# martinruenz/co-fusion

Hardware: AMD Instinct MI355X
Metric: frames/sec at 640x480 (N active models) + ICP-reduce achieved HBM GB/s vs peak (higher is better)
Workload: dtype f32

## Files before the change

### co_fusion_amd/csrc/cabi.hip

```cpp
#include <math.h>
#include <stdio.h>
#include <stdlib.h>
#include <string.h>

#include <string>
#include <vector>

#include "cf_host.h"
#include "gn_ref_host.h"

using namespace cf;

#define HIPCHK(ctx, call)                                                                      \
    do {                                                                                       \
        hipError_t e_ = (call);                                                                \
        if (e_ != hipSuccess) {                                                                \
            (ctx)->set_error(std::string(#call) + ": " + hipGetErrorString(e_));               \
            return CF_EHIP;                                                                    \
        }                                                                                      \
    } while (0)

#define LAUNCHCHK(ctx) HIPCHK(ctx, hipGetLastError())

void cf_ctx::set_error(const std::string& m)
// ... 641 lines not shown
    }
    LAUNCHCHK(ctx);
    return CF_OK;
}

static int populate_rgbd(cf_odom* od, const uint8_t* rgba, float* const* depths, uint8_t* const* images)
{
    cf_ctx* ctx = od->ctx; hipStream_t s = ctx->stream;
    RgbdBatch b{};
    b.c[0] = rgbd_chain(od, rgba, depths, images);
    launch_rgbd_pyramids(s, b, 1, ctx->cfg.width, ctx->cfg.height, od->maxDepthRGB);
    LAUNCHCHK(ctx);
    return CF_OK;
}
int cf_odom_init_rgb_model(cf_odom* od, const uint8_t* pred_rgba) { if (!od || !pred_rgba) return CF_EINVAL; return populate_rgbd(od, pred_rgba, od->lastDepth, od->lastImage); }
int cf_odom_init_rgb(cf_odom* od, const uint8_t* rgba) { if (!od || !rgba) return CF_EINVAL; od->next_depth_is_last = false; return populate_rgbd(od, rgba, od->nextDepth, od->nextImage); }

int cf_odom_init_models_batch(cf_ctx* ctx, cf_odom* const* ods, int n, const float* const* pred_v4, const float* const* pred_n4,
                              const uint8_t* const* pred_rgba, const float* const* poses, const uint8_t* frame_rgba)
{
    if (!ctx || n <= 0 || !frame_rgba) return CF_EINVAL;
    std::vector<const uint8_t*> frames((size_t)n, frame_rgba);
    return cf_odom_init_models_batch_frames(ctx, ods, n, pred_v4, pred_n4, pred_rgba, poses, frames.data());
}

int cf_odom_init_models_batch_frames(cf_ctx* ctx, cf_odom* const* ods, int n, const float* const* pred_v4, const float* const* pred_n4,
                                     const uint8_t* const* pred_rgba, const float* const* poses, const uint8_t* const* frame_rgba)
{
    return cf_odom_init_models_batch_select(ctx, ods, n, pred_v4, pred_n4, pred_rgba, nullptr, nullptr, nullptr, nullptr, 0.f, poses, frame_rgba);
}

// ... 23 lines not shown
        RgbdBatch rb{};
        for (int k = 0; k < nb; k++) {
            cf_odom* od = ods[base + k];
            if (!od || !pred_v4[base + k] || !pred_n4[base + k] || !pred_rgba[base + k] || !poses[base + k] || !frame_rgba[base + k]) return CF_EINVAL;
            mb.m[k] = model_maps_args(od, pred_v4[base + k], pred_n4[base + k], poses[base + k]);
            rb.c[k] = rgbd_chain(od, pred_rgba[base + k], od->lastDepth, od->lastImage);
            rb.c[k].v4 = pred_v4[base + k];
            if (choose && fill_counts[base + k]) {
                if (!alt_v4[base + k] || !alt_n4[base + k] || !alt_rgba[base + k]) return CF_EINVAL;
                mb.m[k].alt_v4 = alt_v4[base + k]; mb.m[k].alt_n4 = alt_n4[base + k]; mb.m[k].sel = fill_counts[base + k]; mb.m[k].sel_ratio = ratio;
                rb.c[k].alt_v4 = alt_v4[base + k]; rb.c[k].alt_rgba = alt_rgba[base + k]; rb.c[k].sel = fill_counts[base + k]; rb.c[k].sel_ratio = ratio;
            }
            od->next_depth_is_last = true;
        }
        int n_chains = nb;
        for (int k = 0; k < nb; k++) {
            cf_odom* od = ods[base + k];
            int owner = -1;
            for (int j = nb; j < n_chains; j++)
                if (rb.c[j].rgba == frame_rgba[base + k]) { owner = j; break; }
            if (owner < 0) {
                owner = n_chains++;
                rb.c[owner] = rgbd_chain(od, frame_rgba[base + k], od->nextDepth, od->nextImage);
                for (int i = 0; i < CF_NUM_PYRS; ++i) rb.c[owner].depth[i] = nullptr;
            }
            rb.fan_owner[k] = (signed char)(owner + 1);
            for (int i = 0; i < CF_NUM_PYRS; ++i) rb.fan_image[i][k] = od->nextImage[i];
        }
        launch_model_maps_and_pyramids(s, mb, nb, rb, n_chains, W, H, ods[base]->maxDepthRGB);
    }
    LAUNCHCHK(ctx);
    return CF_OK;
}

int cf_odom_init_first_rgb(cf_odom* od, const uint8_t* rgba)
{
    if (!od || !rgba) return CF_EINVAL;
    cf_ctx* ctx = od->ctx; hipStream_t s = ctx->stream;
    const int W = ctx->cfg.width, H = ctx->cfg.height;
    launch_intensity(s, rgba, W, H, od->lastNextImage[0]);
// ... 129 lines not shown
    const float t[3] = {pose[3], pose[7], pose[11]};
    memcpy(h->Rprev, R, 36); memcpy(h->tprev, t, 12); memcpy(h->Rcurr, R, 36); memcpy(h->tcurr, t, 12);
    inv33f_host(R, h->Rprev_inv);
    memset(&h->stats, 0, sizeof(h->stats));
    h->solves = 0;
    {
        const int its = (opts->fast_odom ? 3 : 10) + (opts->pyramid ? 9 : 0);
        od->expected_solves = its;
    }
    od->pending_so3_swap = opts->so3 != 0;
    od->launch_shape = LaunchShape{};
    LAUNCHCHK(ctx);
    return CF_OK;
}

static void fill_rgb_args(cf_ctx* ctx, cf_odom* const* ods, int n, RgbArgs out[3])
{
    const cf_cam intr{ctx->cfg.fx, ctx->cfg.fy, ctx->cfg.cx, ctx->cfg.cy};
    for (int l = 0; l < 3; l++) {
        RgbArgs& a = out[l];
        memset(&a, 0, sizeof(a));
        const int div = 1 << l;
        a.cols = ctx->cfg.width >> l; a.rows = ctx->cfg.height >> l;
        a.il = cf_cam{intr.fx / div, intr.fy / div, intr.cx / div, intr.cy / div};
        a.sobelScale = ods[0]->sobelScale; a.maxDepthDelta = ods[0]->maxDepthDeltaRGB;
        for (int m = 0; m < n; m++) {
            a.m[m] = rgb_model_args(ods[m]->h_state, ods[m]->d_state, l);
            a.m[m].no_counts = (ods[m]->band_end > 0 && !ods[m]->band_counts) ? 1 : 0;
            a.m[m].res_blocks = a.m[m].res_range ? residual_blocks_for(ods[m]->res_hint[l]) : 0;
        }
// ... 46 lines not shown
        }
    }
    if (ctx->icp_arith == CF_ICP_ARITH_REFERENCE) {
        for (int m = 0; m < n; m++)
            if (ods[m]->band_end > 0) { ctx->set_error("the reference-order arithmetic (cf_set_icp_arith 2) does not split a tracker's reductions over GPUs"); return CF_ESTATE; }
        RgbPrepBatch rp{};
        for (int base = 0; base < n; base += kPrepBatch) {
            const int nb = n - base < kPrepBatch ? n - base : kPrepBatch;
            rp = RgbPrepBatch{};
            for (int m = base; m < base + nb; m++) {
                if (int r = odom_prepare(ods[m], poses_in[m], opts, err_surfaces ? err_surfaces[m] : nullptr, &rp.m[m - base])) return r;
                ods[m]->h_state->cull = 0; ods[m]->h_state->res_range = nullptr; rp.m[m - base].res_range = nullptr;
                ods[m]->box_hint[0] = kNoBoxHint;
                HIPCHK(ctx, hipMemsetAsync(ods[m]->aabb, 0, 8 * sizeof(unsigned), ctx->stream));
            }
            if (want_rgb) launch_rgb_prep(ctx->stream, rp, nb, ctx->cfg.width, ctx->cfg.height);
        }
        LAUNCHCHK(ctx);
        for (int m = 0; m < n; m++)
            if (int r = ref_track(ctx, ods[m], poses_in[m], opts, err_surfaces ? err_surfaces[m] : nullptr)) return r;
        for (int m = 0; m < n; m++) ods[m]->result_pending = true;
        return CF_OK;
    }
    for (int m = 0; m < n; m++)
        if (ods[m]->gn_epoch_seen != ctx->gn_mode_epoch) {
            HIPCHK(ctx, hipMemsetAsync(ods[m]->rgb_acc, 0, sizeof(unsigned long long) * ods[m]->rgb_acc_words, ctx->stream));
            ods[m]->gn_epoch_seen = ctx->gn_mode_epoch;
        }
    const bool prep_fused = want_rgb && opts->so3 != 0 && n <= kPrepBatch;
    RgbPrepBatch prep{};
    for (int base = 0; base < n; base += kPrepBatch) {
        const int nb = n - base < kPrepBatch ? n - base : kPrepBatch;
        if (base) prep = RgbPrepBatch{};
        for (int m = base; m < base + nb; m++) {
            if (int r = odom_prepare(ods[m], poses_in[m], opts, err_surfaces ? err_surfaces[m] : nullptr, &prep.m[m - base])) return r;
        }
        if (want_rgb && !prep_fused) launch_rgb_prep(ctx->stream, prep, nb, ctx->cfg.width, ctx->cfg.height);
    }
    if (prep_fused) rgb_prep_levels(prep, n, ctx->cfg.width, ctx->cfg.height);
    TrackerStates states{};
    for (int m = 0; m < n; m++) { states.dev[m] = ods[m]->d_state; states.host[m] = ods[m]->h_state; }
    const bool so3_here = opts->so3 != 0;
    const bool icp = !opts->rgb_only && opts->icp_weight > 0;
    const bool rgb = opts->rgb_only || opts->icp_weight < 100;
    IcpArgs icp_args[3];
    fill_icp_args(ctx, ods, n, icp_args);
    RgbArgs rgb_args[3];
    fill_rgb_args(ctx, ods, n, rgb_args);
    OdomDev* h_states[kMaxBatch];
    for (int m = 0; m < n; m++) h_states[m] = ods[m]->h_state;
    GnHook hook{};
// ... 79 lines not shown
    if (!od) return CF_EINVAL;
    cf_ctx* ctx = od->ctx;
    if (int r = cf_wait_stream(ctx)) return r;
    od->result_pending = false;
    if (trans) memcpy(trans, od->h_state->tcurr, 12);
    if (rot) memcpy(rot, od->h_state->Rcurr, 36);
    if (stats) *stats = od->h_state->stats;
    bool fault = od->h_state->stats.fault != 0;
    if (ctx->icp_arith != CF_ICP_ARITH_REFERENCE && od->expected_solves >= 0 && od->h_state->solves != od->expected_solves) {
        (void)hipMemsetAsync(ctx->d_so3_sync, 0, sizeof(So3Sync) * ((size_t)ctx->cfg.max_models + 1), ctx->stream);
        fault = true;
    }
    od->expected_solves = -1;
    if (od->pending_so3_swap) {
        for (int i = 0; i < CF_NUM_PYRS; i++) std::swap(od->lastNextImage[i], od->nextImage[i]);
        od->pending_so3_swap = false;
    }
    if (fault) {
        ctx->set_error("tracking: a bounded device-side wait expired (workgroups of one launch were not co-resident)");
        return CF_ESTATE;
    }
    return CF_OK;
}

int cf_odom_get_covariance(const cf_track_stats* stats, double cov[36])
{
    if (!stats || !cov) return CF_EINVAL;
    constexpr int N = 6;
    double lu[N * N];
    int perm[N];
// ... 141 lines not shown
```

### co_fusion_amd/csrc/cf_host.h

```cpp
#pragma once

#include <mutex>
#include <string>

#include "cf_kernels.h"

struct cf_ctx;
struct cf_thread_binding { const cf_ctx* ctx = nullptr; hipStream_t stream = nullptr; };
extern thread_local cf_thread_binding cf_tls_binding;

struct cf_ctx {
    cf_config cfg{};
    hipStream_t stream = nullptr;
    hipStream_t cur() const { return cf_tls_binding.ctx == this ? cf_tls_binding.stream : stream; }
    hipStream_t own_stream = nullptr;
    std::string last_error;
    std::mutex error_mutex;
    cf::IcpLaunch icp_launch{256, 0};
    int icp_arith = 0;
    float* d_ref = nullptr;
    float* h_ref = nullptr;
    unsigned long long* d_acc_a = nullptr;
    unsigned long long* d_acc_b = nullptr;
    unsigned long long* d_out = nullptr;
    unsigned long long* h_out = nullptr;
    cf::OdomDev* d_scratch_state = nullptr;
    cf::OdomDev* h_scratch_state = nullptr;
    uint8_t* d_cand_scratch = nullptr;
    cf::So3Sync* d_so3_sync = nullptr;
    unsigned gn_mode_epoch = 0;
    int xcd_round_robin = -1;
    int gn_mode = 1;
    static constexpr int kStateSlots = 256;
    cf::OdomDev* d_state_pool = nullptr;
    cf::OdomDev* h_state_pool = nullptr;
    bool slot_used[kStateSlots]{};
    hipEvent_t batch_event = nullptr;
    static constexpr int kLanes = 8;
    hipStream_t lanes[kLanes]{};
    hipEvent_t lane_done[kLanes]{};
    hipEvent_t fork_point = nullptr;
    static constexpr int kMarks = 64;
    hipEvent_t marks[kMarks]{};
    bool mark_set[kMarks]{};
// ... 32 lines not shown
    float* nmap_g_prev[3]{};
    float* vmap_curr[3]{};
    float* nmap_curr[3]{};
    const float* ext_vmap_curr[3]{};
    const float* ext_nmap_curr[3]{};
    float2* zrange[3]{};
    bool zrange_valid = false;
    const float2* ext_zrange[3]{};
    float* lastDepth[3]{};
    float* nextDepth[3]{};
    bool next_depth_is_last = false;
    float* next_depth(int i) const { return next_depth_is_last ? lastDepth[i] : nextDepth[i]; }
    uint8_t* lastImage[3]{};
    uint8_t* nextImage[3]{};
    uint8_t* lastNextImage[3]{};
    int16_t* dIdx[3]{};
    int16_t* dIdy[3]{};
    float* cloud[3]{};
    cf_dataterm* corres[3]{};
    uint8_t* cand[3]{};
    unsigned char* occ = nullptr;
    bool occ_valid = false;
    bool use_occ = false;
    unsigned* aabb = nullptr;
    float map_pose[12]{};
    int box_hint[4] = {0x7fffffff, 0, 0, 0};
    unsigned* res_range = nullptr;
    int res_hint[3] = {-1, -1, -1};
    bool box_valid = false;
    int band_begin = 0, band_end = 0;
// ... 17 lines not shown
```

### co_fusion_amd/csrc/cf_kernels.h

```cpp
#pragma once

#include <hip/hip_runtime.h>
#include <hip/hip_ext.h>
#include <stdint.h>

#include "../../include/cofusion_hip.h"

namespace cf {

constexpr int kGroups = 64;

struct alignas(64) GnHot {
    int icp, level_done; float cull_z[2];
    float Rcurr[9], tcurr[3];
    float Rprev_inv[9], tprev[3];
    int cull_box[4];
    int rgb, rgbOnly, level_done2, pad;
    float krkInv[9], kt[3];
};
static_assert(sizeof(GnHot) == 192, "three 64-byte lines");

struct OdomDev;
struct OdomDev {
    const float* vmap_curr[3];
// ... 74 lines not shown
    const uint8_t* nextImage[3]; const float* nextDepth[3]; const float* lastDepth[3];
    int16_t* dIdx[3]; int16_t* dIdy[3]; uint8_t* cand[3]; float* cloud[3];
    float minScale[3], fx_inv[3], fy_inv[3], cx[3], cy[3];
    unsigned* res_range;
};
struct ModelMapsArgs {
    const float* pred_v4; const float* pred_n4;
    const float* alt_v4; const float* alt_n4;
    const unsigned* sel; float sel_ratio;
    float* snapshot;
    float* vmap[3]; float* nmap[3];
    int cols, rows;
    float R[9], t[3];
    unsigned char* occ;
    unsigned* aabb;
};
constexpr int kPrepBatch = 8;
struct ModelMapsBatch { ModelMapsArgs m[kPrepBatch]; };
struct RgbPrepBatch { RgbPrepArgs m[kPrepBatch]; };
struct RgbdChain {
    const float* v4; const uint8_t* rgba; float* depth[3]; uint8_t* image[3];
    const float* alt_v4; const uint8_t* alt_rgba; const unsigned* sel; float sel_ratio;
};
struct RgbdBatch {
    RgbdChain c[2 * kPrepBatch];
    uint8_t* fan_image[3][kPrepBatch];
    signed char fan_owner[kPrepBatch];
};
void launch_model_maps(hipStream_t s, const ModelMapsBatch& b, int n);
void launch_frame_maps(hipStream_t s, FrameMapsArgs a, int W, int H);
void launch_rgbd_pyramids(hipStream_t s, const RgbdBatch& b, int n_chains, int W, int H, float cutoff);
void launch_model_maps_and_pyramids(hipStream_t s, const ModelMapsBatch& mb, int n, const RgbdBatch& rb, int n_chains, int W, int H, float cutoff);
void launch_rgb_prep(hipStream_t s, RgbPrepBatch b, int n, int W, int H);

struct IDiv { unsigned M, s; };
inline IDiv make_idiv(int d)
{
    if (d < 2) return IDiv{0x80000000u, 0u};
    unsigned l = 0;
    while ((1u << l) < (unsigned)d) l++;
    return IDiv{(unsigned)((((unsigned long long)1 << (31 + l)) + (unsigned)d - 1) / (unsigned)d), l - 1};
}
constexpr int kGramBits[8] = {20, 20, 20, 17, 17, 17, 22, 0};
struct LaunchShape { int icp[3]; int res[3]; int icp_err; };
struct IcpLaunch { int threads; int ppt; int gram;
                   LaunchShape* const* shape = nullptr; };

// ... 218 lines not shown
```

### co_fusion_amd/csrc/track_prep.hip

```cpp
#include "cf_device.h"
#include "cf_kernels.h"
#include "track_prep_dev.h"

namespace cf {

static constexpr int kBlock = 256;
static inline int grid_for(int n) { return (n + kBlock - 1) / kBlock; }

__global__ void __launch_bounds__(kBlock) vmap_kernel(const float* __restrict__ depth, int cols, int rows, float fx_inv,
                                                      float fy_inv, float cx, float cy, float cutoff,
                                                      float* __restrict__ vmap)
{
    const int i = blockIdx.x * kBlock + threadIdx.x;
    if (i >= cols * rows) return;
    const int v = i / cols, u = i - v * cols;
    const float z = depth[i];
    if (z != 0 && z < cutoff) {
        vmap[i] = z * (u - cx) * fx_inv;
        vmap[i + rows * cols] = z * (v - cy) * fy_inv;
        vmap[i + 2 * rows * cols] = z;
    } else {
        vmap[i] = qnan();
    }
}
// ... 190 lines not shown
    const float4* __restrict__ v4 = reinterpret_cast<const float4*>(alt ? c.alt_v4 : c.v4);
    const uchar4* __restrict__ rgba = reinterpret_cast<const uchar4*>(alt ? c.alt_rgba : c.rgba);
    const int nb = (N + kBlock - 1) / kBlock;
    if (bx < nb) {
        const int i = bx * kBlock + threadIdx.x;
        if (i >= N || !c.depth[0]) return;
        const float z = v4[i].z;
        c.depth[0][i] = (z > cutoff || z <= 0) ? qnan() : z;
    } else {
        const int i = (bx - nb) * kBlock + threadIdx.x;
        if (i >= N) return;
        const uchar4 s = rgba[i];
        rgbd_store_image(b, by, 0, i, (uint8_t)(int)((float)s.x * 0.114f + (float)s.y * 0.299f + (float)s.z * 0.587f));
    }
}
__global__ void __launch_bounds__(kBlock) rgbd_base_kernel(const RgbdBatch b, int N, float cutoff) { rgbd_base_body(b, N, cutoff, (int)blockIdx.x, (int)blockIdx.y); }
__global__ void __launch_bounds__(kBlock) rgbd_pyrdown_kernel(const RgbdBatch b, int level, int scols, int srows)
{
    const RgbdChain& c = b.c[blockIdx.y];
    const int n = (scols / 2) * (srows / 2), nb = (n + kBlock - 1) / kBlock;
    if ((int)blockIdx.x < nb) {
        const int i = blockIdx.x * kBlock + threadIdx.x;
        if (i < n && c.depth[level]) pyrdown_f32_px(c.depth[level], scols, srows, c.depth[level + 1], i);
    } else {
        const int i = (blockIdx.x - nb) * kBlock + threadIdx.x;
        if (i < n) rgbd_store_image(b, (int)blockIdx.y, level + 1, i, pyrdown_u8_val(c.image[level], scols, srows, i));
    }
}

__global__ void __launch_bounds__(kBlock) rgb_expand_kernel(const uint8_t* __restrict__ rgb, int N, uchar4* __restrict__ rgba)
// ... 97 lines not shown
    }
    if (edge) { nmap[i] = qnan(); return; }
    const float x01 = (z01 != 0 && z01 < cutoff) ? z01 * ((u + 1) - cx) * fx_inv : qnan();
    const float x10 = (z10 != 0 && z10 < cutoff) ? z10 * (u - cx) * fx_inv : qnan();
    if (!is_nan(x00) && !is_nan(x01) && !is_nan(x10)) {
        const f3 v00 = {x00, z * (v - cy) * fy_inv, z};
        const f3 v01 = {x01, z01 * (v - cy) * fy_inv, z01};
        const f3 v10 = {x10, z10 * ((v + 1) - cy) * fy_inv, z10};
        const f3 r = normalized(cross(v01 - v00, v10 - v00));
        nmap[i] = r.x; nmap[i + N] = r.y; nmap[i + 2 * N] = r.z;
    } else {
        nmap[i] = qnan();
    }
}

__global__ void __launch_bounds__(kBlock) rgb_prep_kernel(const RgbPrepBatch b) { rgb_prep_body(b.m[blockIdx.y], (int)blockIdx.x); }

struct MapVal { f3 p; bool have; };

__device__ __forceinline__ void emit_map(float* __restrict__ map, int idx, int N, const MapVal& m, const m33& R, const f3& t, bool add_t)
{
    if (!m.have) { map[idx] = qnan(); return; }
    if (!is_nan(m.p.x)) {
        f3 d = mul(R, m.p);
        if (add_t) d = d + t;
        map[idx] = d.x; map[idx + N] = d.y; map[idx + 2 * N] = d.z;
    } else {
        map[idx] = qnan(); map[idx + N] = m.p.y; map[idx + 2 * N] = m.p.z;
    }
}

// ... 71 lines not shown
    const int cols = a.cols, rows = a.rows, N0 = cols * rows, c1 = cols >> 1, c2 = cols >> 2, N1 = N0 >> 2, N2 = N0 >> 4;
    const int lane = threadIdx.x & 63, lx = lane & 15, ly = lane >> 4;
    const int tiles_x = cols >> 4;
    const int tile = bx * 4 + (threadIdx.x >> 6);
    if (tile >= tiles_x * (rows >> 2)) return;
    const int ty = tile / tiles_x, tx = tile - ty * tiles_x;
    const int x = tx * 16 + lx, y = ty * 4 + ly, i0 = y * cols + x;
    const bool alt = a.sel && (float)a.sel[0] / (float)a.sel[1] < a.sel_ratio;
    const float4* __restrict__ v4 = reinterpret_cast<const float4*>(alt ? a.alt_v4 : a.pred_v4);
    const float4* __restrict__ n4 = reinterpret_cast<const float4*>(alt ? a.alt_n4 : a.pred_n4);
    float4* __restrict__ snap = reinterpret_cast<float4*>(a.snapshot);
    m33 R; for (int k = 0; k < 9; k++) R.m[k] = a.R[k];
    const f3 tr = {a.t[0], a.t[1], a.t[2]};
    const float4 vs = v4[i0], ns = n4[i0];
    snap[i0] = vs;
    MapVal v0, n0;
    v0.have = true; n0.have = true;
    const bool valid = !(vs.z == 0);
    if (valid) { v0.p = f3{vs.x, vs.y, vs.z}; n0.p = f3{ns.x, ns.y, ns.z}; }
    else { v0.p = f3{qnan(), qnan(), qnan()}; n0.p = v0.p; }
    emit_map(a.vmap[0], i0, N0, v0, R, tr, true);
    emit_map(a.nmap[0], i0, N0, n0, R, tr, false);
    const MapVal v01 = lane_mapval(v0, lane + 1), v10 = lane_mapval(v0, lane + 16), v11 = lane_mapval(v0, lane + 17);
    const MapVal n01 = lane_mapval(n0, lane + 1), n10 = lane_mapval(n0, lane + 16), n11 = lane_mapval(n0, lane + 17);
    MapVal v1, n1;
    v1.have = false; n1.have = false; v1.p = f3{qnan(), qnan(), qnan()}; n1.p = v1.p;
    if (((lx | ly) & 1) == 0) {
        v1 = resize4(v0, v01, v10, v11, false);
        n1 = resize4(n0, n01, n10, n11, true);
        const int i1 = (y >> 1) * c1 + (x >> 1);
// ... 15 lines not shown
        const float inf = __int_as_float(0x7f800000);
        float lo[3] = {inf, inf, inf}, hi[3] = {-inf, -inf, -inf};
        if (valid && !is_nan(v0.p.x) && !is_nan(vs.z)) { lo[0] = hi[0] = (float)x; lo[1] = hi[1] = (float)y; lo[2] = hi[2] = vs.z; }
#pragma unroll
        for (int o = 32; o > 0; o >>= 1)
#pragma unroll
            for (int k = 0; k < 3; k++) { lo[k] = fminf(lo[k], __shfl_xor(lo[k], o, 64)); hi[k] = fmaxf(hi[k], __shfl_xor(hi[k], o, 64)); }
        if (lane < 6 && lo[0] <= hi[0] && lo[1] <= hi[1] && lo[2] <= hi[2]) {
            const float val = lane == 0 ? lo[0] : lane == 1 ? lo[1] : lane == 2 ? lo[2] : lane == 3 ? hi[0] : lane == 4 ? hi[1] : hi[2];
            const unsigned key = lane < 3 ? ~fkey(val) : fkey(val);
            if (key > __hip_atomic_load(&a.aabb[lane], __ATOMIC_RELAXED, __HIP_MEMORY_SCOPE_AGENT)) atomicMax(&a.aabb[lane], key);
        }
    }
}
__global__ void __launch_bounds__(256) model_maps_tiled_kernel(const ModelMapsBatch b) { model_maps_tiled_body(b, (int)blockIdx.x, (int)blockIdx.y); }
__global__ void __launch_bounds__(256) prep_fused_kernel(const ModelMapsBatch mb, int mm_bx, int mm_total, const RgbdBatch rb, int N, float cutoff, int rb_bx)
{
    const int b = blockIdx.x;
    if (b < mm_total) { const int by = b / mm_bx; model_maps_tiled_body(mb, b - by * mm_bx, by); }
    else { const int r = b - mm_total, by = r / rb_bx; rgbd_base_body(rb, N, cutoff, r - by * rb_bx, by); }
}

static Level3 levels3(int W, int H)
{
    Level3 L; int acc = 0;
    for (int i = 0; i < 3; i++) { L.cols[i] = W >> i; L.rows[i] = H >> i; acc += grid_for(L.cols[i] * L.rows[i]); L.blk_end[i] = acc; }
    return L;
}
void launch_frame_maps(hipStream_t s, FrameMapsArgs a, int W, int H)
{
    a.L = levels3(W, H);
    frame_maps_kernel<<<a.L.blk_end[2], kBlock, 0, s>>>(a);
}
void rgb_prep_levels(RgbPrepBatch& b, int n, int W, int H)
{
    const Level3 L = levels3(W, H);
    for (int m = 0; m < n; m++) b.m[m].L = L;
}
void launch_rgb_prep(hipStream_t s, RgbPrepBatch b, int n, int W, int H)
{
    const Level3 L = levels3(W, H);
    for (int m = 0; m < n; m++) b.m[m].L = L;
    rgb_prep_kernel<<<dim3(L.blk_end[2], n), kBlock, 0, s>>>(b);
}
void launch_model_maps(hipStream_t s, const ModelMapsBatch& b, int n)
{
    const int cols = b.m[0].cols, rows = b.m[0].rows;
    if (cols % 16 == 0 && rows % 4 == 0) {
        const int tiles = (cols >> 4) * (rows >> 2);
        model_maps_tiled_kernel<<<dim3((tiles + 3) / 4, n), 256, 0, s>>>(b);
        return;
    }
    const int t = (cols >> 2) * (rows >> 2);
    model_maps_kernel<<<dim3((t + 63) / 64, n), 64, 0, s>>>(b);
}
void launch_model_maps_and_pyramids(hipStream_t s, const ModelMapsBatch& mb, int n, const RgbdBatch& rb, int n_chains, int W, int H, float cutoff)
{
    static_assert(kBlock == 256, "the fused launch runs both bodies with 256 threads");
    const int cols = mb.m[0].cols, rows = mb.m[0].rows;
    if (cols % 16 == 0 && rows % 4 == 0) {
        const int mm_bx = ((cols >> 4) * (rows >> 2) + 3) / 4, rb_bx = 2 * grid_for(W * H);
        prep_fused_kernel<<<mm_bx * n + rb_bx * n_chains, 256, 0, s>>>(mb, mm_bx, mm_bx * n, rb, W * H, cutoff, rb_bx);
    } else {
        launch_model_maps(s, mb, n);
        rgbd_base_kernel<<<dim3(2 * grid_for(W * H), n_chains), kBlock, 0, s>>>(rb, W * H, cutoff);
    }
    for (int i = 0; i + 1 < 3; i++)
        rgbd_pyrdown_kernel<<<dim3(2 * grid_for(((W >> i) / 2) * ((H >> i) / 2)), n_chains), kBlock, 0, s>>>(rb, i, W >> i, H >> i);
}
void launch_rgbd_pyramids(hipStream_t s, const RgbdBatch& b, int n_chains, int W, int H, float cutoff)
{
    rgbd_base_kernel<<<dim3(2 * grid_for(W * H), n_chains), kBlock, 0, s>>>(b, W * H, cutoff);
    for (int i = 0; i + 1 < 3; i++)
        rgbd_pyrdown_kernel<<<dim3(2 * grid_for(((W >> i) / 2) * ((H >> i) / 2)), n_chains), kBlock, 0, s>>>(b, i, W >> i, H >> i);
}
void launch_vmap(hipStream_t s, const float* depth, int cols, int rows, cf_cam intr, float cutoff, float* vmap)
{
// ... 55 lines not shown
```

### co_fusion_amd/csrc/track_prep_dev.h

```cpp
#pragma once
#include "cf_device.h"
#include "cf_kernels.h"

namespace cf {
__device__ __forceinline__ int level_of(const Level3& L, int b, int& lb)
{
    const int lv = b < L.blk_end[0] ? 0 : (b < L.blk_end[1] ? 1 : 2);
    lb = b - (lv ? L.blk_end[lv - 1] : 0);
    return lv;
}

__device__ __forceinline__ void rgb_prep_body(const RgbPrepArgs& a, int bx)
{
    int lb;
    const int lv = level_of(a.L, bx, lb);
    const int cols = a.L.cols[lv], rows = a.L.rows[lv];
    const int k = lb * 256 + (int)threadIdx.x;
    uint8_t ok = 0;
    if (k < cols * rows) {
    const int y = k / cols, x = k - y * cols;
    const uint8_t* __restrict__ src = a.nextImage[lv];
    {
        const float z = a.lastDepth[lv][k];
        float* __restrict__ cloud3 = a.cloud[lv];
        cloud3[k * 3 + 0] = (x - a.cx[lv]) * z * a.fx_inv[lv];
        cloud3[k * 3 + 1] = (y - a.cy[lv]) * z * a.fy_inv[lv];
        cloud3[k * 3 + 2] = z;
    }
    float dxv = 0, dyv = 0;
    constexpr float sx[9] = {0.52201f, 0.00000f, -0.52201f, 0.79451f, -0.00000f, -0.79451f, 0.52201f, 0.00000f, -0.52201f};
    constexpr float sy[9] = {0.52201f, 0.79451f, 0.52201f, 0.00000f, 0.00000f, 0.00000f, -0.52201f, -0.79451f, -0.52201f};
    if (x >= 1 && y >= 1 && x <= cols - 2 && y <= rows - 2) {
        const uint8_t* __restrict__ p0 = src + (y - 1) * cols + (x - 1);
#pragma unroll
        for (int r = 0; r < 3; r++)
#pragma unroll
            for (int c = 0; c < 3; c++) {
                const float s = (float)p0[r * cols + c];
                dxv += s * sx[8 - (r * 3 + c)];
                dyv += s * sy[8 - (r * 3 + c)];
            }
    } else {
        int kk = 8;
        for (int j = max(y - 1, 0); j <= min(y + 1, rows - 1); j++)
            for (int c = max(x - 1, 0); c <= min(x + 1, cols - 1); c++) {
                const float s = (float)src[j * cols + c];
                dxv += s * sx[kk];
                dyv += s * sy[kk];
                --kk;
            }
    }
    const int16_t dx16 = (int16_t)(int)dxv, dy16 = (int16_t)(int)dyv;
    a.dIdx[lv][k] = dx16; a.dIdy[lv][k] = dy16;
    if (x < cols - 5 && y < rows - 1) {
        bool valid = true;
        for (int u = max(y - 2, 0); u < min(y + 2, rows); u++)
            for (int v = max(x - 2, 0); v < min(x + 2, cols); v++) valid = valid && (src[u * cols + v] > 0);
        if (valid) {
            const int valx = dx16, valy = dy16;
            const float mTwo = (float)((valx * valx) + (valy * valy));
            if (mTwo >= a.minScale[lv] && !is_nan(a.nextDepth[lv][k])) ok = 1;
        }
    }
    a.cand[lv][k] = ok;
    }
    if (a.res_range) {
        if (__syncthreads_or(ok)) {
            if (threadIdx.x == 0) { atomicMax(&a.res_range[2 * lv], ~(unsigned)lb); atomicMax(&a.res_range[2 * lv + 1], (unsigned)lb + 1u); }
        }
    }
}
}
```

### co_fusion_amd/csrc/track_reduce.hip

```cpp
#include "cf_device.h"
#include "cf_kernels.h"
#include "track_prep_dev.h"
#include "track_sums_dev.h"

namespace cf {

__device__ __forceinline__ int idiv(int n, IDiv d) { return (int)(__umulhi((unsigned)n, d.M) >> d.s); }

struct IcpProj { f3 vcurr_g; int g; int inb; int ux, uy; };

__device__ __forceinline__ IcpProj icp_project(const m33& Rcurr, const f3& tcurr, const m33& Rprev_inv, const f3& tprev, const cf_cam& intr,
                                               int cols, int rows, f3 vcurr)
{
    IcpProj o;
    o.vcurr_g = mul(Rcurr, vcurr) + tcurr;
    const f3 vcurr_cp = mul(Rprev_inv, o.vcurr_g - tprev);
    const int ux = f2i_rn(vcurr_cp.x * intr.fx / vcurr_cp.z + intr.cx);
    const int uy = f2i_rn(vcurr_cp.y * intr.fy / vcurr_cp.z + intr.cy);
    o.inb = !(ux < 0 || uy < 0 || ux >= cols || uy >= rows || vcurr_cp.z < 0);
    o.g = o.inb ? uy * cols + ux : 0;
    o.ux = o.inb ? ux : 0; o.uy = o.inb ? uy : 0;
    return o;
}

// ... 672 lines not shown

bool launch_gn_track(hipStream_t s, IcpLaunch cfg, const TrackerStates& states, So3Sync* so3_syncs, const GnHook* hook, const IcpArgs icp_args[3],
                     const RgbArgs rgb_args[3], int n, int width, int height, bool so3, bool pyramid, bool fast_odom, bool rgb, bool icp, int mode,
                     ProfSink* prof, OdomDev* const* h_states, const RgbPrepBatch* prep)
{
    int iterations[3];
    iterations[0] = fast_odom ? 3 : 10;
    iterations[1] = pyramid ? 5 : 0;
    iterations[2] = pyramid ? 4 : 0;
    int first_level = 2;
    while (first_level > 0 && iterations[first_level] == 0) first_level--;
    {
        const int gx = so3 ? 8 * kSo3Blocks : 1;
        static const RgbPrepBatch none{};
        const int prep_bx = prep ? prep->m[0].L.blk_end[2] : 0;
        so3_prealign_kernel<<<gx * n + prep_bx * n, 256, 0, s>>>(states, so3_syncs, so3 ? 1 : 0, first_level, gx, gx * n, prep ? *prep : none, prep_bx);
    }
    GnArgs gn{};
    gn.icp_gram = cfg.gram;
    gn.slot_px = cfg.threads * 4;
    for (int m = 0; m < n; m++) {
        gn.od[m] = const_cast<OdomDev*>(icp_args[0].m[m].st);
        gn.icp_acc[m] = icp_args[0].m[m].acc;
        gn.rgb_acc[m] = rgb_args[0].m[m].rgb_acc;
        gn.od_host[m] = h_states ? h_states[m] : nullptr;
    }
    const bool slots = mode != 0;
    bool any_culled = false;
    for (int m = 0; m < n; m++) any_culled = any_culled || (icp_args[0].m[m].cull && icp_args[0].m[m].err);
    const bool err_aside = icp && any_culled;
    bool hook_failed = false;
// ... 207 lines not shown
```

### co_fusion_amd/csrc/track_so3_dev.h

```cpp
#pragma once
#include "track_prep_dev.h"
#include "track_sums_dev.h"

namespace cf {

__device__ __forceinline__ cf_cam cam_level(cf_cam c, int level)
{
    const int div = 1 << level;
    return cf_cam{c.fx / div, c.fy / div, c.cx / div, c.cy / div};
}

__device__ __forceinline__ void screen_box(const float* lo, const float* hi, const float* Rb, const float* tb, const float* Rcurr, const float* tcurr,
                                           cf_cam intr, float distThres, int W, int H, int lane, int (&out)[4], float (&zout)[2])
{
    const float finf = __int_as_float(0x7f800000);
    zout[0] = -finf; zout[1] = finf;
    if (!(lo[0] <= hi[0])) { out[0] = 1; out[1] = 1; out[2] = 0; out[3] = 0; return; }
    const float m = distThres * 1.01f + 1e-3f;
    const float px = (lane & 1) ? hi[0] + 3.f : lo[0] - 3.f, py = (lane & 2) ? hi[1] + 3.f : lo[1] - 3.f;
    const float znear = lo[2] - m, pz = (lane & 4) ? hi[2] + m : znear;
    const float cx_ = (px - intr.cx) / intr.fx * pz, cy_ = (py - intr.cy) / intr.fy * pz;
    const float dx = (Rb[0] * cx_ + Rb[1] * cy_ + Rb[2] * pz + tb[0]) - tcurr[0];
    const float dy = (Rb[3] * cx_ + Rb[4] * cy_ + Rb[5] * pz + tb[1]) - tcurr[1];
    const float dz = (Rb[6] * cx_ + Rb[7] * cy_ + Rb[8] * pz + tb[2]) - tcurr[2];
// ... 121 lines not shown
    __shared__ unsigned long long totals[16];
    so3_pass(lastImage, nextImage, B, Ki, krlr.m, cols, rows, lds, totals, blockIdx.x, gridDim.x);
    if (threadIdx.x < 16) out16[threadIdx.x] = totals[threadIdx.x];
}

#ifdef CF_ABLATE
__device__ unsigned long long g_so3_trace[12][8];
#define OSTAMP(it, k) do { if (lead && by == 0 && threadIdx.x == 0) g_so3_trace[it][k] = wall_clock64(); } while (0)
#else
#define OSTAMP(it, k) do {} while (0)
#endif
__global__ void __launch_bounds__(256) so3_prealign_kernel(const TrackerStates ts, So3Sync* __restrict__ syncs, int do_so3,
                                                           int first_level, int gx, int so3_blocks, const RgbPrepBatch prep, int prep_bx)
{
    if ((int)blockIdx.x >= so3_blocks) {
        const int r = (int)blockIdx.x - so3_blocks, m = r / prep_bx;
        rgb_prep_body(prep.m[m], r - m * prep_bx);
        return;
    }
    const int by = (int)blockIdx.x / gx, bxx = (int)blockIdx.x - by * gx;
    OdomDev* const god = ts.dev[by];
    So3Sync* sync = syncs + by;
    __shared__ OdomDev s_od;
    __shared__ unsigned long long lds[16][16];
    __shared__ unsigned long long totals[16];
    __shared__ float s_basis[9], s_kinv[9], s_krlr[9];
    __shared__ int s_done;
    __shared__ double s_resultR[9];
    __shared__ double s_K[9], s_Kinv[9];
    __shared__ float s_Rlr[9];
    __shared__ float s_lastError, s_lastCount;
    __shared__ double s_lastResultR[9];
// ... 146 lines not shown
```

Measured before the change: 902.8.

## Share Sobel gradients across models with the same frame; fold depth copy into model maps

Tags each model's next-image pyramid with a per-chain sequence number so RGB prep can group models that share the same source frame. Only one block grid per group computes the Sobel gradients and the validity window, then loops over the member models to write their clouds, gradients and candidate masks. Separately, the fused prep kernel now writes the level-0 thresholded depth from the model-maps body and runs only an intensity pass for RGBD chains, which halves that grid. This adds host-side grouping bookkeeping and per-model serial work inside each block, and correctness depends on the tags being reset whenever images are swapped.

```diff
diff --git a/co_fusion_amd/csrc/cabi.hip b/co_fusion_amd/csrc/cabi.hip
--- a/co_fusion_amd/csrc/cabi.hip
+++ b/co_fusion_amd/csrc/cabi.hip
@@ -679,7 +679,7 @@
     return CF_OK;
 }
 int cf_odom_init_rgb_model(cf_odom* od, const uint8_t* pred_rgba) { if (!od || !pred_rgba) return CF_EINVAL; return populate_rgbd(od, pred_rgba, od->lastDepth, od->lastImage); }
-int cf_odom_init_rgb(cf_odom* od, const uint8_t* rgba) { if (!od || !rgba) return CF_EINVAL; od->next_depth_is_last = false; return populate_rgbd(od, rgba, od->nextDepth, od->nextImage); }
+int cf_odom_init_rgb(cf_odom* od, const uint8_t* rgba) { if (!od || !rgba) return CF_EINVAL; od->next_depth_is_last = false; od->next_image_tag = 0; return populate_rgbd(od, rgba, od->nextDepth, od->nextImage); }
 
 int cf_odom_init_models_batch(cf_ctx* ctx, cf_odom* const* ods, int n, const float* const* pred_v4, const float* const* pred_n4,
                               const uint8_t* const* pred_rgba, const float* const* poses, const uint8_t* frame_rgba)
@@ -733,6 +733,7 @@
             od->next_depth_is_last = true;
         }
         int n_chains = nb;
+        unsigned long long chain_tag[2 * kPrepBatch] = {};
         for (int k = 0; k < nb; k++) {
             cf_odom* od = ods[base + k];
             int owner = -1;
@@ -742,7 +743,9 @@
                 owner = n_chains++;
                 rb.c[owner] = rgbd_chain(od, frame_rgba[base + k], od->nextDepth, od->nextImage);
                 for (int i = 0; i < CF_NUM_PYRS; ++i) rb.c[owner].depth[i] = nullptr;
+                chain_tag[owner] = ++ctx->image_tag_seq;
             }
+            od->next_image_tag = chain_tag[owner];
             rb.fan_owner[k] = (signed char)(owner + 1);
             for (int i = 0; i < CF_NUM_PYRS; ++i) rb.fan_image[i][k] = od->nextImage[i];
         }
@@ -902,6 +905,13 @@
     return CF_OK;
 }
 
+static void prep_group(RgbPrepBatch& b, cf_odom* const* ods, int n)
+{
+    unsigned long long tags[kPrepBatch];
+    for (int m = 0; m < n; m++) tags[m] = ods[m]->next_image_tag;
+    rgb_prep_group(b, n, tags);
+}
+
 static void fill_rgb_args(cf_ctx* ctx, cf_odom* const* ods, int n, RgbArgs out[3])
 {
     const cf_cam intr{ctx->cfg.fx, ctx->cfg.fy, ctx->cfg.cx, ctx->cfg.cy};
@@ -978,7 +988,7 @@
                 ods[m]->box_hint[0] = kNoBoxHint;
                 HIPCHK(ctx, hipMemsetAsync(ods[m]->aabb, 0, 8 * sizeof(unsigned), ctx->stream));
             }
-            if (want_rgb) launch_rgb_prep(ctx->stream, rp, nb, ctx->cfg.width, ctx->cfg.height);
+            if (want_rgb) { prep_group(rp, ods + base, nb); launch_rgb_prep(ctx->stream, rp, nb, ctx->cfg.width, ctx->cfg.height); }
         }
         LAUNCHCHK(ctx);
         for (int m = 0; m < n; m++)
@@ -999,6 +1009,7 @@
         for (int m = base; m < base + nb; m++) {
             if (int r = odom_prepare(ods[m], poses_in[m], opts, err_surfaces ? err_surfaces[m] : nullptr, &prep.m[m - base])) return r;
         }
+        if (want_rgb) prep_group(prep, ods + base, nb);
         if (want_rgb && !prep_fused) launch_rgb_prep(ctx->stream, prep, nb, ctx->cfg.width, ctx->cfg.height);
     }
     if (prep_fused) rgb_prep_levels(prep, n, ctx->cfg.width, ctx->cfg.height);
@@ -1108,6 +1119,7 @@
     od->expected_solves = -1;
     if (od->pending_so3_swap) {
         for (int i = 0; i < CF_NUM_PYRS; i++) std::swap(od->lastNextImage[i], od->nextImage[i]);
+        od->next_image_tag = 0;
         od->pending_so3_swap = false;
     }
     if (fault) {
diff --git a/co_fusion_amd/csrc/cf_host.h b/co_fusion_amd/csrc/cf_host.h
--- a/co_fusion_amd/csrc/cf_host.h
+++ b/co_fusion_amd/csrc/cf_host.h
@@ -28,6 +28,7 @@
     cf::OdomDev* h_scratch_state = nullptr;
     uint8_t* d_cand_scratch = nullptr;
     cf::So3Sync* d_so3_sync = nullptr;
+    unsigned long long image_tag_seq = 0;
     unsigned gn_mode_epoch = 0;
     int xcd_round_robin = -1;
     int gn_mode = 1;
@@ -90,6 +91,7 @@
     uint8_t* lastImage[3]{};
     uint8_t* nextImage[3]{};
     uint8_t* lastNextImage[3]{};
+    unsigned long long next_image_tag = 0;
     int16_t* dIdx[3]{};
     int16_t* dIdy[3]{};
     float* cloud[3]{};
diff --git a/co_fusion_amd/csrc/cf_kernels.h b/co_fusion_amd/csrc/cf_kernels.h
--- a/co_fusion_amd/csrc/cf_kernels.h
+++ b/co_fusion_amd/csrc/cf_kernels.h
@@ -112,10 +112,16 @@
     float R[9], t[3];
     unsigned char* occ;
     unsigned* aabb;
+    float* depth0; float depth_cutoff;
 };
 constexpr int kPrepBatch = 8;
 struct ModelMapsBatch { ModelMapsArgs m[kPrepBatch]; };
-struct RgbPrepBatch { RgbPrepArgs m[kPrepBatch]; };
+struct RgbPrepBatch {
+    RgbPrepArgs m[kPrepBatch];
+    int n, n_groups;
+    unsigned char group_lead[kPrepBatch];
+    unsigned char lead_of[kPrepBatch];
+};
 struct RgbdChain {
     const float* v4; const uint8_t* rgba; float* depth[3]; uint8_t* image[3];
     const float* alt_v4; const uint8_t* alt_rgba; const unsigned* sel; float sel_ratio;
@@ -129,6 +135,7 @@
 void launch_frame_maps(hipStream_t s, FrameMapsArgs a, int W, int H);
 void launch_rgbd_pyramids(hipStream_t s, const RgbdBatch& b, int n_chains, int W, int H, float cutoff);
 void launch_model_maps_and_pyramids(hipStream_t s, const ModelMapsBatch& mb, int n, const RgbdBatch& rb, int n_chains, int W, int H, float cutoff);
+void rgb_prep_group(RgbPrepBatch& b, int n, const unsigned long long* tags);
 void launch_rgb_prep(hipStream_t s, RgbPrepBatch b, int n, int W, int H);
 
 struct IDiv { unsigned M, s; };
diff --git a/co_fusion_amd/csrc/track_prep.hip b/co_fusion_amd/csrc/track_prep.hip
--- a/co_fusion_amd/csrc/track_prep.hip
+++ b/co_fusion_amd/csrc/track_prep.hip
@@ -228,6 +228,16 @@
         rgbd_store_image(b, by, 0, i, (uint8_t)(int)((float)s.x * 0.114f + (float)s.y * 0.299f + (float)s.z * 0.587f));
     }
 }
+__device__ __forceinline__ void rgbd_intensity_body(const RgbdBatch& b, int N, int bx, int by)
+{
+    const RgbdChain& c = b.c[by];
+    const bool alt = c.sel && (float)c.sel[0] / (float)c.sel[1] < c.sel_ratio;
+    const uchar4* __restrict__ rgba = reinterpret_cast<const uchar4*>(alt ? c.alt_rgba : c.rgba);
+    const int i = bx * kBlock + threadIdx.x;
+    if (i >= N) return;
+    const uchar4 s = rgba[i];
+    rgbd_store_image(b, by, 0, i, (uint8_t)(int)((float)s.x * 0.114f + (float)s.y * 0.299f + (float)s.z * 0.587f));
+}
 __global__ void __launch_bounds__(kBlock) rgbd_base_kernel(const RgbdBatch b, int N, float cutoff) { rgbd_base_body(b, N, cutoff, (int)blockIdx.x, (int)blockIdx.y); }
 __global__ void __launch_bounds__(kBlock) rgbd_pyrdown_kernel(const RgbdBatch b, int level, int scols, int srows)
 {
@@ -355,7 +365,7 @@
     }
 }
 
-__global__ void __launch_bounds__(kBlock) rgb_prep_kernel(const RgbPrepBatch b) { rgb_prep_body(b.m[blockIdx.y], (int)blockIdx.x); }
+__global__ void __launch_bounds__(kBlock) rgb_prep_kernel(const RgbPrepBatch b) { rgb_prep_body(b, (int)blockIdx.y, (int)blockIdx.x); }
 
 struct MapVal { f3 p; bool have; };
 
@@ -457,6 +467,7 @@
     const f3 tr = {a.t[0], a.t[1], a.t[2]};
     const float4 vs = v4[i0], ns = n4[i0];
     snap[i0] = vs;
+    if (a.depth0) a.depth0[i0] = (vs.z > a.depth_cutoff || vs.z <= 0) ? qnan() : vs.z;
     MapVal v0, n0;
     v0.have = true; n0.have = true;
     const bool valid = !(vs.z == 0);
@@ -502,11 +513,11 @@
     }
 }
 __global__ void __launch_bounds__(256) model_maps_tiled_kernel(const ModelMapsBatch b) { model_maps_tiled_body(b, (int)blockIdx.x, (int)blockIdx.y); }
-__global__ void __launch_bounds__(256) prep_fused_kernel(const ModelMapsBatch mb, int mm_bx, int mm_total, const RgbdBatch rb, int N, float cutoff, int rb_bx)
+__global__ void __launch_bounds__(256) prep_fused_kernel(const ModelMapsBatch mb, int mm_bx, int mm_total, const RgbdBatch rb, int N, int rb_bx)
 {
     const int b = blockIdx.x;
     if (b < mm_total) { const int by = b / mm_bx; model_maps_tiled_body(mb, b - by * mm_bx, by); }
-    else { const int r = b - mm_total, by = r / rb_bx; rgbd_base_body(rb, N, cutoff, r - by * rb_bx, by); }
+    else { const int r = b - mm_total, by = r / rb_bx; rgbd_intensity_body(rb, N, r - by * rb_bx, by); }
 }
 
 static Level3 levels3(int W, int H)
@@ -525,11 +536,23 @@
     const Level3 L = levels3(W, H);
     for (int m = 0; m < n; m++) b.m[m].L = L;
 }
+void rgb_prep_group(RgbPrepBatch& b, int n, const unsigned long long* tags)
+{
+    b.n = n; b.n_groups = 0;
+    for (int t = 0; t < n; t++) {
+        int lead = t;
+        if (tags && tags[t])
+            for (int j = 0; j < t; j++)
+                if (tags[j] == tags[t]) { lead = j; break; }
+        b.lead_of[t] = (unsigned char)lead;
+        if (lead == t) b.group_lead[b.n_groups++] = (unsigned char)t;
+    }
+}
 void launch_rgb_prep(hipStream_t s, RgbPrepBatch b, int n, int W, int H)
 {
     const Level3 L = levels3(W, H);
     for (int m = 0; m < n; m++) b.m[m].L = L;
-    rgb_prep_kernel<<<dim3(L.blk_end[2], n), kBlock, 0, s>>>(b);
+    rgb_prep_kernel<<<dim3(L.blk_end[2], b.n_groups), kBlock, 0, s>>>(b);
 }
 void launch_model_maps(hipStream_t s, const ModelMapsBatch& b, int n)
 {
@@ -547,8 +570,10 @@
     static_assert(kBlock == 256, "the fused launch runs both bodies with 256 threads");
     const int cols = mb.m[0].cols, rows = mb.m[0].rows;
     if (cols % 16 == 0 && rows % 4 == 0) {
-        const int mm_bx = ((cols >> 4) * (rows >> 2) + 3) / 4, rb_bx = 2 * grid_for(W * H);
-        prep_fused_kernel<<<mm_bx * n + rb_bx * n_chains, 256, 0, s>>>(mb, mm_bx, mm_bx * n, rb, W * H, cutoff, rb_bx);
+        const int mm_bx = ((cols >> 4) * (rows >> 2) + 3) / 4, rb_bx = grid_for(W * H);
+        ModelMapsBatch m = mb;
+        for (int k = 0; k < n; k++) { m.m[k].depth0 = rb.c[k].depth[0]; m.m[k].depth_cutoff = cutoff; }
+        prep_fused_kernel<<<mm_bx * n + rb_bx * n_chains, 256, 0, s>>>(m, mm_bx, mm_bx * n, rb, W * H, rb_bx);
     } else {
         launch_model_maps(s, mb, n);
         rgbd_base_kernel<<<dim3(2 * grid_for(W * H), n_chains), kBlock, 0, s>>>(rb, W * H, cutoff);
diff --git a/co_fusion_amd/csrc/track_prep_dev.h b/co_fusion_amd/csrc/track_prep_dev.h
--- a/co_fusion_amd/csrc/track_prep_dev.h
+++ b/co_fusion_amd/csrc/track_prep_dev.h
@@ -10,63 +10,70 @@
     return lv;
 }
 
-__device__ __forceinline__ void rgb_prep_body(const RgbPrepArgs& a, int bx)
+__device__ __forceinline__ void rgb_prep_body(const RgbPrepBatch& b, int group, int bx)
 {
+    const int lead = b.group_lead[group];
+    const RgbPrepArgs& a0 = b.m[lead];
     int lb;
-    const int lv = level_of(a.L, bx, lb);
-    const int cols = a.L.cols[lv], rows = a.L.rows[lv];
+    const int lv = level_of(a0.L, bx, lb);
+    const int cols = a0.L.cols[lv], rows = a0.L.rows[lv];
     const int k = lb * 256 + (int)threadIdx.x;
-    uint8_t ok = 0;
-    if (k < cols * rows) {
+    const bool in = k < cols * rows;
     const int y = k / cols, x = k - y * cols;
-    const uint8_t* __restrict__ src = a.nextImage[lv];
-    {
-        const float z = a.lastDepth[lv][k];
-        float* __restrict__ cloud3 = a.cloud[lv];
-        cloud3[k * 3 + 0] = (x - a.cx[lv]) * z * a.fx_inv[lv];
-        cloud3[k * 3 + 1] = (y - a.cy[lv]) * z * a.fy_inv[lv];
-        cloud3[k * 3 + 2] = z;
-    }
-    float dxv = 0, dyv = 0;
-    constexpr float sx[9] = {0.52201f, 0.00000f, -0.52201f, 0.79451f, -0.00000f, -0.79451f, 0.52201f, 0.00000f, -0.52201f};
-    constexpr float sy[9] = {0.52201f, 0.79451f, 0.52201f, 0.00000f, 0.00000f, 0.00000f, -0.52201f, -0.79451f, -0.52201f};
-    if (x >= 1 && y >= 1 && x <= cols - 2 && y <= rows - 2) {
-        const uint8_t* __restrict__ p0 = src + (y - 1) * cols + (x - 1);
+    int16_t dx16 = 0, dy16 = 0;
+    bool window = false;
+    if (in) {
+        const uint8_t* __restrict__ src = a0.nextImage[lv];
+        float dxv = 0, dyv = 0;
+        constexpr float sx[9] = {0.52201f, 0.00000f, -0.52201f, 0.79451f, -0.00000f, -0.79451f, 0.52201f, 0.00000f, -0.52201f};
+        constexpr float sy[9] = {0.52201f, 0.79451f, 0.52201f, 0.00000f, 0.00000f, 0.00000f, -0.52201f, -0.79451f, -0.52201f};
+        if (x >= 1 && y >= 1 && x <= cols - 2 && y <= rows - 2) {
+            const uint8_t* __restrict__ p0 = src + (y - 1) * cols + (x - 1);
 #pragma unroll
-        for (int r = 0; r < 3; r++)
+            for (int r = 0; r < 3; r++)
 #pragma unroll
-            for (int c = 0; c < 3; c++) {
-                const float s = (float)p0[r * cols + c];
-                dxv += s * sx[8 - (r * 3 + c)];
-                dyv += s * sy[8 - (r * 3 + c)];
-            }
-    } else {
-        int kk = 8;
-        for (int j = max(y - 1, 0); j <= min(y + 1, rows - 1); j++)
-            for (int c = max(x - 1, 0); c <= min(x + 1, cols - 1); c++) {
-                const float s = (float)src[j * cols + c];
-                dxv += s * sx[kk];
-                dyv += s * sy[kk];
-                --kk;
-            }
-    }
-    const int16_t dx16 = (int16_t)(int)dxv, dy16 = (int16_t)(int)dyv;
-    a.dIdx[lv][k] = dx16; a.dIdy[lv][k] = dy16;
-    if (x < cols - 5 && y < rows - 1) {
-        bool valid = true;
-        for (int u = max(y - 2, 0); u < min(y + 2, rows); u++)
-            for (int v = max(x - 2, 0); v < min(x + 2, cols); v++) valid = valid && (src[u * cols + v] > 0);
-        if (valid) {
-            const int valx = dx16, valy = dy16;
-            const float mTwo = (float)((valx * valx) + (valy * valy));
-            if (mTwo >= a.minScale[lv] && !is_nan(a.nextDepth[lv][k])) ok = 1;
+                for (int c = 0; c < 3; c++) {
+                    const float s = (float)p0[r * cols + c];
+                    dxv += s * sx[8 - (r * 3 + c)];
+                    dyv += s * sy[8 - (r * 3 + c)];
+                }
+        } else {
+            int kk = 8;
+            for (int j = max(y - 1, 0); j <= min(y + 1, rows - 1); j++)
+                for (int c = max(x - 1, 0); c <= min(x + 1, cols - 1); c++) {
+                    const float s = (float)src[j * cols + c];
+                    dxv += s * sx[kk];
+                    dyv += s * sy[kk];
+                    --kk;
+                }
+        }
+        dx16 = (int16_t)(int)dxv; dy16 = (int16_t)(int)dyv;
+        if (x < cols - 5 && y < rows - 1) {
+            window = true;
+            for (int u = max(y - 2, 0); u < min(y + 2, rows); u++)
+                for (int v = max(x - 2, 0); v < min(x + 2, cols); v++) window = window && (src[u * cols + v] > 0);
         }
     }
-    a.cand[lv][k] = ok;
-    }
-    if (a.res_range) {
-        if (__syncthreads_or(ok)) {
-            if (threadIdx.x == 0) { atomicMax(&a.res_range[2 * lv], ~(unsigned)lb); atomicMax(&a.res_range[2 * lv + 1], (unsigned)lb + 1u); }
+    const int valx = dx16, valy = dy16;
+    const float mTwo = (float)((valx * valx) + (valy * valy));
+    for (int t = lead; t < b.n; t++) {
+        if (b.lead_of[t] != lead) continue;
+        const RgbPrepArgs& a = b.m[t];
+        uint8_t ok = 0;
+        if (in) {
+            const float z = a.lastDepth[lv][k];
+            float* __restrict__ cloud3 = a.cloud[lv];
+            cloud3[k * 3 + 0] = (x - a.cx[lv]) * z * a.fx_inv[lv];
+            cloud3[k * 3 + 1] = (y - a.cy[lv]) * z * a.fy_inv[lv];
+            cloud3[k * 3 + 2] = z;
+            a.dIdx[lv][k] = dx16; a.dIdy[lv][k] = dy16;
+            if (window && mTwo >= a.minScale[lv] && !is_nan(a.nextDepth[lv][k])) ok = 1;
+            a.cand[lv][k] = ok;
+        }
+        if (a.res_range) {
+            if (__syncthreads_or(ok)) {
+                if (threadIdx.x == 0) { atomicMax(&a.res_range[2 * lv], ~(unsigned)lb); atomicMax(&a.res_range[2 * lv + 1], (unsigned)lb + 1u); }
+            }
         }
     }
 }
diff --git a/co_fusion_amd/csrc/track_reduce.hip b/co_fusion_amd/csrc/track_reduce.hip
--- a/co_fusion_amd/csrc/track_reduce.hip
+++ b/co_fusion_amd/csrc/track_reduce.hip
@@ -710,7 +710,7 @@
         const int gx = so3 ? 8 * kSo3Blocks : 1;
         static const RgbPrepBatch none{};
         const int prep_bx = prep ? prep->m[0].L.blk_end[2] : 0;
-        so3_prealign_kernel<<<gx * n + prep_bx * n, 256, 0, s>>>(states, so3_syncs, so3 ? 1 : 0, first_level, gx, gx * n, prep ? *prep : none, prep_bx);
+        so3_prealign_kernel<<<gx * n + prep_bx * (prep ? prep->n_groups : 0), 256, 0, s>>>(states, so3_syncs, so3 ? 1 : 0, first_level, gx, gx * n, prep ? *prep : none, prep_bx);
     }
     GnArgs gn{};
     gn.icp_gram = cfg.gram;
diff --git a/co_fusion_amd/csrc/track_so3_dev.h b/co_fusion_amd/csrc/track_so3_dev.h
--- a/co_fusion_amd/csrc/track_so3_dev.h
+++ b/co_fusion_amd/csrc/track_so3_dev.h
@@ -159,8 +159,8 @@
                                                            int first_level, int gx, int so3_blocks, const RgbPrepBatch prep, int prep_bx)
 {
     if ((int)blockIdx.x >= so3_blocks) {
-        const int r = (int)blockIdx.x - so3_blocks, m = r / prep_bx;
-        rgb_prep_body(prep.m[m], r - m * prep_bx);
+        const int r = (int)blockIdx.x - so3_blocks, g = r / prep_bx;
+        rgb_prep_body(prep, g, r - g * prep_bx);
         return;
     }
     const int by = (int)blockIdx.x / gx, bxx = (int)blockIdx.x - by * gx;
```

Result: no change. 914.4 (median of 6 runs) (+1.3%).
